# hherlyng/knp-emi-cgx

Hardware: AMD Instinct MI355X
Metric: MDoF/s per implicit timestep (assembly+GMRES) (higher is better)
Workload: dtype f64

## Files before the change

include/knpemi_hip.h:

```cpp
#ifndef KNPEMI_HIP_H
#define KNPEMI_HIP_H

#include <stdint.h>

#ifdef __cplusplus
extern "C" {
#endif

#define KNP_MAX_IONS 3
#define KNP_MAX_AUX 8
#define KNP_DIAG_MAX_CONSTS 64
#define KNP_MAX_PROG_REGS 48
#define KNP_MAX_AMG_LEVELS 16

#define KNP_OK 0
#define KNP_E_ARG (-1)
#define KNP_E_HIP (-2)
#define KNP_E_STATE (-3)
#define KNP_E_ALLOC (-4)
#define KNP_E_MESH (-5)

#define KNP_CONVERGED_RTOL 2
#define KNP_CONVERGED_ATOL 3
#define KNP_DIVERGED_ITS (-3)
// ... 131 lines not shown
int knp_amg_reset(knp_ctx* ctx, int32_t hier, int32_t n_levels, int32_t pre_sweeps, int32_t post_sweeps, int32_t cheby_degree);
int knp_amg_set_node_fields(knp_ctx* ctx, int32_t hier, int32_t nf);
int knp_amg_set_level(knp_ctx* ctx, int32_t hier, int32_t level, int32_t n_rows, int32_t n_cols_halo,
                      const int32_t* A_rowptr, const int32_t* A_colind, const double* A_vals,
                      const double* inv_diag, double lambda_max,
                      int32_t n_coarse,
                      const int32_t* P_rowptr, const int32_t* P_colind, const double* P_vals,
                      const int32_t* R_rowptr, const int32_t* R_colind, const double* R_vals);
int knp_amg_set_level_prolongator(knp_ctx* ctx, int32_t hier, int32_t level, int32_t n_rows_P, const int32_t* P_rp,
                                  const int32_t* P_ci, const double* P_v);
int knp_amg_set_level_mode(knp_ctx* ctx, int32_t hier, int32_t level, int32_t distributed, int32_t repl_n);
int knp_amg_set_coarse(knp_ctx* ctx, int32_t hier, int32_t n, const double* dense_inverse );
int knp_amg_set_level_smoothed(knp_ctx* ctx, int32_t hier, int32_t level, int32_t n_rows, const int32_t* S_rowptr, const int32_t* S_colind,
                        const double* S_vals);
int knp_amg_set_level_coarse_fused(knp_ctx* ctx, int32_t hier, int32_t level, int32_t Rt_rows, const int32_t* Rt_rowptr, const int32_t* Rt_colind,
                                   const double* Rt_vals, int32_t U_rows, const int32_t* U_rowptr, const int32_t* U_colind, const double* U_vals);
int knp_amg_use_native_level0(knp_ctx* ctx, int32_t hier, int32_t mode);
int knp_amg_set_precision(knp_ctx* ctx, int32_t fp32_storage);
int knp_gmres_prepare(knp_ctx* ctx, const double* b);
int knp_gmres_solve(knp_ctx* ctx, const double* b, double* x, double rtol, double atol, int32_t max_it,
                    int32_t restart, int32_t* its, double* rnorm, int32_t* reason);
int knp_fgmres_prepare(knp_ctx* ctx, const double* b);
int knp_fgmres_solve(knp_ctx* ctx, const double* b, double* x, double rtol, double atol, int32_t max_it,
                     int32_t restart, int32_t* its, double* rnorm, int32_t* reason);

int knp_pack(knp_ctx* ctx, const knp_fields_out* fields, double* x);
int knp_unpack(knp_ctx* ctx, const double* x, const knp_fields_out* fields);
int knp_hh_update(knp_ctx* ctx, const double* phi_m, double* n, double* m, double* h, int32_t count,
                  double dt, double phi_rest, int32_t rush_larsen, int32_t substeps);
int knp_l2_norms(knp_ctx* ctx, const double* phi_i, const double* phi_e, double* out );
int knp_diag_set_cell_tags(knp_ctx* ctx, int32_t n_tags, const int32_t* seg_ptr ,
                           const int32_t* cells );
int knp_diag_volume_integrals(knp_ctx* ctx, const knp_fields* fields, double* out );
int knp_diag_set_facet_tags(knp_ctx* ctx, int32_t n_tags, const int32_t* seg_ptr ,
                            const int32_t* facets );
int knp_diag_set_program(knp_ctx* ctx, int32_t n_instr, const int32_t* code , int32_t n_consts,
                         const double* consts );
int knp_diag_set_program_constants(knp_ctx* ctx, int32_t n_consts, const double* consts );
int knp_diag_membrane_integral(knp_ctx* ctx, const knp_fields* fields, double* out );

int knp_timer_mark(knp_ctx* ctx, int32_t join_assembly);
int knp_timer_read(knp_ctx* ctx, int32_t capacity, double* seconds , int32_t* n_intervals);
int knp_timer_pending(const knp_ctx* ctx);
int knp_profile_enable(knp_ctx* ctx, int32_t class_mask);
int knp_profile_get(knp_ctx* ctx, int32_t cls, double* ms, int64_t* launches);
int knp_profile_reset(knp_ctx* ctx);
enum { KNP_ST_BNORM = 0 , KNP_ST_ALLREDUCE = 1 ,
       KNP_ST_HALO = 2 , KNP_ST_READBACK = 3 ,
       KNP_ST_FUSED = 4 ,
       KNP_ST_NORM_FALLBACK = 5 ,
       KNP_ST_BLOCKED = 6 ,
       KNP_ST_FUSED_LEVELS = 7 ,
       KNP_ST_FUSED_DOTS = 8 ,
       KNP_ST_SPMV_DOTS = 9 , KNP_ST_COUNT = 10 };
int knp_get_stats(const knp_ctx* ctx, double* out );
int knp_get_traffic_model(const knp_ctx* ctx, double* out );

#ifdef __cplusplus
}
#endif
#endif
```

knp-emi-cgx_amd/cgx_hip/backend.py:

```python
from __future__ import annotations

import ctypes as C
import os

import numpy as np
import torch

from . import _lib
from ._lib import Fields, FieldsOut, KnpError, MeshDesc
from .parallel import HaloPlan, all_reduce_sum_, guarded


class _CAI:

    def __init__(self, ptr, n):
        self.__cuda_array_interface__ = {"shape": (int(n),), "typestr": "<f8", "data": (int(ptr), False),
                                         "version": 2, "strides": None}


def _f64(a):
    return a.ctypes.data_as(_lib.f64p)


def _i32(a):
# ... 543 lines not shown
        self.check(self.lib.knp_pc_set_coupled_potential(self.ctx, 1 if on else 0))

    def precond_phi_csr(self, embedded=True):
        import scipy.sparse as sp
        sz = (C.c_int64 * _lib.KNP_SZ_COUNT)()
        self.check(self.lib.knp_get_sizes(self.ctx, sz))
        nnz = sz[_lib.SZ_NNZ_P_PHI]
        no = self.n_nodes_owned
        rp = np.empty(no + 1, dtype=np.int32)
        ci = np.empty(nnz, dtype=np.int32)
        va = np.empty(nnz, dtype=np.float64)
        self.check(self.lib.knp_get_precond_phi_csr(self.ctx, _i32(rp), _i32(ci), _f64(va)))
        if not embedded:
            M = sp.csr_matrix((va, ci, rp), shape=(no, self.n_nodes))
            M.sort_indices()
            return M
        keep = va != 0.0
        node_of_entry = np.repeat(np.arange(no, dtype=np.int32), np.diff(rp))
        cnt = np.bincount(node_of_entry[keep], minlength=no)
        indptr = np.zeros(self.n_dof_owned + 1, dtype=np.int64)
        indptr[4 * np.arange(no, dtype=np.int64) + 4] = cnt
        np.cumsum(indptr, out=indptr)
        idx_t = np.int32 if max(int(indptr[-1]), self.n_dof_local) < 2 ** 31 - 1 else np.int64
        M = sp.csr_matrix((va[keep], (4 * ci[keep].astype(idx_t) + 3), indptr.astype(idx_t)), shape=(self.n_dof_owned, self.n_dof_local))
        M.sort_indices()
        return M

    def timer_mark(self, join_assembly=False):
        self.check(self.lib.knp_timer_mark(self.ctx, 1 if join_assembly else 0))

    def timer_pending(self):
        return int(self.lib.knp_timer_pending(self.ctx))

    def timer_read(self):
        n = self.timer_pending()
        if n < 2:
            if n:
                out = (C.c_double * 1)()
                k = C.c_int32()
                self.check(self.lib.knp_timer_read(self.ctx, 1, out, C.byref(k)))
            return np.zeros(0)
        out = (C.c_double * n)()
        k = C.c_int32()
        self.check(self.lib.knp_timer_read(self.ctx, n, out, C.byref(k)))
        return np.array(out[:k.value], dtype=np.float64)

    def profile_enable(self, mask=0x1f):
        self.check(self.lib.knp_profile_enable(self.ctx, int(mask)))

    def profile_reset(self):
        self.check(self.lib.knp_profile_reset(self.ctx))

    def stats(self):
        out = (C.c_double * 10)()
        self.check(self.lib.knp_get_stats(self.ctx, out))
        return {"bnorm": out[0], "allreduces": int(out[1]), "halos": int(out[2]), "readbacks": int(out[3]), "fused": int(out[4]),
                "norm_fallbacks": int(out[5]), "blocked": int(out[6]), "fused_levels": int(out[7]),
                "fused_dots": int(out[8]), "spmv_dots": int(out[9])}

    def traffic_model(self):
        out = (C.c_double * 5)()
        self.check(self.lib.knp_get_traffic_model(self.ctx, out))
        return {"spmv": out[0], "pc": out[1], "assembly_matrix": out[2], "assembly_rhs": out[3], "vector": out[4]}

    def profile_get(self):
        names = ["spmv", "orthogonalisation", "pc", "assembly", "other"]
        out = {}
        for k, nm in enumerate(names):
            ms = C.c_double()
            n = C.c_int64()
            self.check(self.lib.knp_profile_get(self.ctx, k, C.byref(ms), C.byref(n)))
            out[nm] = (ms.value, n.value)
        return out
```

knp-emi-cgx_amd/csrc/knp_internal.hpp:

```cpp
#pragma once
#include <hip/hip_runtime.h>

#include <cstdint>
#include <string>
#include <vector>

#include "knpemi_hip.h"

#define KNP_NPROF 5

struct KnpHostGraph {
    int dim = 0, nv1 = 0;
    int n_v = 0, n_v_owned = 0, n_c = 0, n_c_owned = 0, n_g = 0, n_q = 0;
    int n_nodes = 0, n_nodes_owned = 0;
    std::vector<int32_t> node_i, node_e;
    std::vector<int32_t> node_vertex;
    std::vector<uint8_t> node_side;
    std::vector<int32_t> pair_ptr;
    std::vector<int32_t> pair_col;
    std::vector<int32_t> pair_row;
    std::vector<double> pair_M, pair_K;
    std::vector<int32_t> contrib_ptr;
    std::vector<int32_t> contrib_cell;
    std::vector<double> contrib_k;
// ... 232 lines not shown
    double *d_w = nullptr, *d_t = nullptr;
    double* d_Z = nullptr;
    int z_cap = 0;
    double* d_partial = nullptr;
    double* d_red = nullptr;
    double* h_red = nullptr;
    double* h_red_dev = nullptr;
    double* mirror() const { return (allreduce && p2p_red < 0) ? nullptr : h_red_dev; }
    int64_t phi_count_cached = -1;
    int64_t* h_seq = nullptr;
    int64_t* h_seq_dev = nullptr;
    int64_t seq_counter = 0;
    int asm_full = 0;
    double asm_dt = -1.0;
    int n_bc = 0;
    int32_t* d_bc_dofs = nullptr;
    int defl_m = 0;
    int32_t* d_defl_mode = nullptr;
    double* d_defl_einv = nullptr;
    double* d_y = nullptr;
    double* d_gm = nullptr;
    int gm_cap = 0;
    int64_t n_norm_fallback = 0;
    int n_red_blocks = 0;
    knp_halo_fn halo = nullptr;
    knp_allreduce_fn allreduce = nullptr;
    knp_level_comm_fn level_comm = nullptr;
    void* comm_user = nullptr;
    KnpP2P* p2p = nullptr;
    int p2p_fine = -1;
    int p2p_red = -1;
    bool hook_allreduce() const { return allreduce && p2p_red < 0; }
    int comm_rc = 0;
    int n_int = 0, n_bnd = 0;
    int32_t *d_nodes_int = nullptr, *d_nodes_bnd = nullptr;
    hipStream_t stream3 = nullptr;
    hipEvent_t ev_x = nullptr, ev_halo = nullptr;
    hipStream_t stream2 = nullptr;
    hipEvent_t ev_fork = nullptr, ev_join = nullptr;
    const double* prep_b = nullptr;
    const double* fprep_b = nullptr;
    int prep_fused = 0;
    int prep_conc = 0;
    bool prep_deferred = false;
    bool side_ws = false;
    double *d_t2_s = nullptr, *d_w2_s = nullptr, *d_wb = nullptr, *d_partial_s = nullptr;
    hipStream_t stream_asm = nullptr;
    hipEvent_t ev_fork_asm = nullptr, ev_asm = nullptr;
    bool asm_pending = false;
    double last_bnorm = 0.0;
    int64_t n_allreduce = 0, n_halo = 0, n_readback = 0;
    int64_t n_fused_dots = 0;
    int64_t n_spmv_dots = 0;
    std::vector<hipEvent_t> tm_events;
    size_t tm_used = 0;
    KnpDiagMap diag_cells, diag_facets;
    int32_t* diag_code = nullptr;
    int diag_n_instr = 0, diag_n_regs = 0, diag_n_consts = 0;
    double diag_consts[KNP_DIAG_MAX_CONSTS] = {};
    bool diag_prog = false;
    int prof_on = 0;
    std::vector<hipEvent_t> prof_pool;
    struct ProfRec { hipEvent_t a, b; int cls; };
    std::vector<ProfRec> prof_recs;
    double prof_ms[KNP_NPROF] = {0, 0, 0, 0, 0};
    int64_t prof_n[KNP_NPROF] = {0, 0, 0, 0, 0};
};

int knp_host_threads();
```

knp-emi-cgx_amd/csrc/knp_kernels.hip:

```cpp
#include <hip/hip_runtime.h>
#include <hip/hip_ext.h>

#include <algorithm>
#include <cmath>
#include <cstdio>
#include <cstdlib>
#include <cstring>
#include <new>

#include "knp_internal.hpp"

#define HIPCHK(call)                                                                       \
    do {                                                                                   \
        hipError_t e_ = (call);                                                            \
        if (e_ != hipSuccess) {                                                            \
            ctx->err = std::string(#call) + ": " + hipGetErrorString(e_);                  \
            return KNP_E_HIP;                                                              \
        }                                                                                  \
    } while (0)
#define KCHK(expr)                         \
    do {                                   \
        int rc_ = (expr);                  \
        if (rc_ != KNP_OK) return rc_;     \
    } while (0)
// ... 1829 lines not shown
    a = block_sum(a, sm);
    if (threadIdx.x == 0) {
        out[slot0 + i] = a;
        if (host_mirror) host_mirror[slot0 + i] = a;
        if (seq) {
            __threadfence_system();
            *seq = seq_val;
        }
    }
}

__global__ void __launch_bounds__(NT) k_dot(int n, const double* __restrict__ a, const double* __restrict__ b,
                                            double* __restrict__ partial) {
    __shared__ double sm[NT / 64];
    double acc = 0.0;
    for (int e = blockIdx.x * NT + threadIdx.x; e < n; e += gridDim.x * NT) acc += a[e] * b[e];
    acc = block_sum(acc, sm);
    if (threadIdx.x == 0) partial[blockIdx.x] = acc;
}

__global__ void __launch_bounds__(NT) k_scale_rsqrt(int n, const double* __restrict__ in, const double* __restrict__ nrm2,
                                                    double* __restrict__ out) {
    const double inv = 1.0 / sqrt(*nrm2);
    for (int e = blockIdx.x * NT + threadIdx.x; e < n; e += gridDim.x * NT) out[e] = in[e] * inv;
}
__global__ void __launch_bounds__(NT) k_scale_rsqrt_proj(int n, const double* __restrict__ in, const double* __restrict__ nrm2,
                                                         const double* __restrict__ phi_sum, double inv_count, double* __restrict__ out,
                                                         double* __restrict__ gm_g = nullptr, int m = 0) {
    if (gm_g && blockIdx.x == 0)
        for (int i = threadIdx.x; i <= m; i += NT) gm_g[i] = (i == 0) ? sqrt(*nrm2) : 0.0;
    const double inv = 1.0 / sqrt(*nrm2);
    const double mean = (*phi_sum) * inv_count;
    for (int e = blockIdx.x * NT + threadIdx.x; e < n; e += gridDim.x * NT) out[e] = ((e & 3) == 3 ? in[e] - mean : in[e]) * inv;
}
__global__ void k_proj_norm(double* __restrict__ red, int slot_s, int slot_out, double inv_count, double cancel, double* mirror,
                            volatile int64_t* seq, int64_t seq_val) {
    if (threadIdx.x != 0) return;
    proj_norm_body(red[slot_s], red[slot_s + 1], red, slot_out, inv_count, cancel, mirror, seq, seq_val);
}
__global__ void __launch_bounds__(NT) k_lincomb(int n, int64_t ldv, int m, const double* __restrict__ V,
                                                const double* __restrict__ y, double* __restrict__ x) {
    for (int e = blockIdx.x * NT + threadIdx.x; e < n; e += gridDim.x * NT) {
        double xe = x[e];
        for (int i = 0; i < m; ++i) xe += y[i] * V[(int64_t)i * ldv + e];
        x[e] = xe;
    }
}

__global__ void k_gm_init(GmLayout L, double* __restrict__ gm, const double* __restrict__ beta2) {
    const int t = threadIdx.x;
    for (int i = t; i <= L.m; i += blockDim.x) gm[L.g() + i] = (i == 0) ? sqrt(*beta2) : 0.0;
}

__global__ void __launch_bounds__(NT)
k_update_scale(int n, int64_t ldv, int m, const double* __restrict__ V, const double* __restrict__ h, const double* __restrict__ w,
               const double* __restrict__ st, double ns_scale, double* __restrict__ out) {
    const double inv = st[1] == 0.0 ? 1.0 / sqrt(st[0]) : 1.0;
    const double mean = ns_scale != 0.0 ? h[m] * ns_scale : 0.0;
    const int n2 = n >> 1;
    for (int e2 = blockIdx.x * NT + threadIdx.x; e2 < n2; e2 += gridDim.x * NT) {
        double2 we = *reinterpret_cast<const double2*>(w + 2 * (size_t)e2);
        if (e2 & 1) we.y -= mean;
        for (int i = 0; i < m; ++i) {
            const double2 v = *reinterpret_cast<const double2*>(V + (int64_t)i * ldv + 2 * (size_t)e2);
            const double hi = h[i];
            we.x -= hi * v.x;
            we.y -= hi * v.y;
        }
        *reinterpret_cast<double2*>(out + 2 * (size_t)e2) = make_double2(we.x * inv, we.y * inv);
    }
}
__global__ void __launch_bounds__(NT) k_scale_inplace_rsqrt(int n, const double* __restrict__ nrm2, double* __restrict__ v) {
    const double inv = 1.0 / sqrt(*nrm2);
    for (int e = blockIdx.x * NT + threadIdx.x; e < n; e += gridDim.x * NT) v[e] *= inv;
}
__global__ void k_gm_solve_y(GmLayout L, int jd, double* __restrict__ gm) {
    if (threadIdx.x != 0) return;
    double* y = gm + L.y();
    const double* g = gm + L.g();
    for (int i = jd - 1; i >= 0; --i) {
        double s = g[i];
        for (int k = i + 1; k < jd; ++k) s -= gm[L.H(i, k)] * y[k];
        y[i] = s / gm[L.H(i, i)];
    }
}

__global__ void __launch_bounds__(NT) k_lincomb_solve(GmLayout L, int jd, double* __restrict__ gm, int n, int64_t ldv,
                                                      const double* __restrict__ V, double* __restrict__ x) {
    __shared__ double sH[8 * 8], sg[8], sy[8];
    if (threadIdx.x < jd * jd) sH[threadIdx.x] = gm[L.H(threadIdx.x % jd, threadIdx.x / jd)];
    if (threadIdx.x < jd) sg[threadIdx.x] = gm[L.g() + threadIdx.x];
    __syncthreads();
    if (threadIdx.x == 0) {
        for (int i = jd - 1; i >= 0; --i) {
            double s = sg[i];
            for (int k = i + 1; k < jd; ++k) s -= sH[i + jd * k] * sy[k];
            sy[i] = s / sH[i + jd * i];
        }
        if (blockIdx.x == 0)
            for (int i = 0; i < jd; ++i) gm[L.y() + i] = sy[i];
    }
    __syncthreads();
    for (int e = blockIdx.x * NT + threadIdx.x; e < n; e += gridDim.x * NT) {
        double xe = x[e];
        for (int i = 0; i < jd; ++i) xe += sy[i] * V[(int64_t)i * ldv + e];
        x[e] = xe;
    }
}

template <bool SOLVE>
__global__ void __launch_bounds__(NT) k_zcorr(GmLayout L, int jd, double* __restrict__ gm, int n, int64_t ldv, const double* __restrict__ Z,
                                              double* __restrict__ t, double* __restrict__ partial) {
    __shared__ double sH[8 * 8], sg[8], sy[8], sm[NT / 64];
    if (SOLVE) {
        if (threadIdx.x < jd * jd) sH[threadIdx.x] = gm[L.H(threadIdx.x % jd, threadIdx.x / jd)];
        if (threadIdx.x < jd) sg[threadIdx.x] = gm[L.g() + threadIdx.x];
        __syncthreads();
        if (threadIdx.x == 0) {
            for (int i = jd - 1; i >= 0; --i) {
                double s = sg[i];
                for (int k = i + 1; k < jd; ++k) s -= sH[i + jd * k] * sy[k];
                sy[i] = s / sH[i + jd * i];
            }
            if (blockIdx.x == 0)
                for (int i = 0; i < jd; ++i) gm[L.y() + i] = sy[i];
        }
        __syncthreads();
    }
    const double* __restrict__ y = SOLVE ? sy : gm + L.y();
    double ps = 0.0;
    for (int e = blockIdx.x * NT + threadIdx.x; e < n; e += gridDim.x * NT) {
        double c = 0.0;
        for (int i = 0; i < jd; ++i) c += y[i] * Z[(int64_t)i * ldv + e];
        t[e] = c;
        if ((e & 3) == 3) ps += c;
    }
    ps = block_sum(ps, sm);
    if (threadIdx.x == 0) partial[blockIdx.x] = ps;
}
__global__ void __launch_bounds__(NT) k_axpy_proj(int n, const double* __restrict__ t, const double* __restrict__ phi_sum, double inv_count,
                                                  double* __restrict__ x) {
    const double mean = (*phi_sum) * inv_count;
    for (int e = blockIdx.x * NT + threadIdx.x; e < n; e += gridDim.x * NT) x[e] += (e & 3) == 3 ? t[e] - mean : t[e];
}

__global__ void __launch_bounds__(NT) k_axpy(int n, double a, const double* __restrict__ x, double* __restrict__ y) {
    for (int e = blockIdx.x * NT + threadIdx.x; e < n; e += gridDim.x * NT) y[e] += a * x[e];
}
__global__ void __launch_bounds__(NT) k_fill(int n, double a, double* __restrict__ y) {
    for (int e = blockIdx.x * NT + threadIdx.x; e < n; e += gridDim.x * NT) y[e] = a;
}
__global__ void __launch_bounds__(NT) k_diag_scale(int n, double a, const double* __restrict__ d,
                                                   const double* __restrict__ x, double* __restrict__ y) {
    for (int e = blockIdx.x * NT + threadIdx.x; e < n; e += gridDim.x * NT) y[e] = a * d[e] * x[e];
}

__global__ void __launch_bounds__(NT) k_phi_sum(int n_nodes, const double* __restrict__ z, double* __restrict__ partial) {
    __shared__ double sm[NT / 64];
    double acc = 0.0;
    for (int n = blockIdx.x * NT + threadIdx.x; n < n_nodes; n += gridDim.x * NT) acc += z[(size_t)4 * n + 3];
// ... 2641 lines not shown
        HIPCHK(hipMemset(ctx->d_gm, 0, (size_t)GL.size() * sizeof(double)));
        ctx->gm_cap = GL.size();
    }
    double* gm = ctx->d_gm;
    auto read_state = [&](double& res_out, int& flag_out) -> int {
        ++ctx->n_readback;
        if (ctx->mirror() && ctx->h_seq_dev) {
            KCHK(read_slots_inner(ctx, GM_RES, 2, ctx->seq_counter));
            if (ctx->p2p) KCHK(knp_p2p_check(ctx));
            res_out = ctx->h_red[GM_RES];
            flag_out = (int)ctx->h_red[GM_RES + 1];
        } else {
            double tmp[3];
            HIPCHK(hipMemcpyAsync(tmp, gm + GL.st(), 3 * sizeof(double), hipMemcpyDeviceToHost, st));
            HIPCHK(hipStreamSynchronize(st));
            res_out = tmp[2];
            flag_out = (int)tmp[1];
        }
        return KNP_OK;
    };

    bool lazy_bnorm = false;
    if (ctx->prep_b == b && restart == ctx->gm_restart && ctx->prep_conc) {
        lazy_bnorm = true;
    } else if (ctx->prep_b == b && restart == ctx->gm_restart) {
        HIPCHK(hipEventSynchronize(ctx->ev_join));
        ctx->prep_b = nullptr;
        if (!ctx->h_red_dev) {
            HIPCHK(hipMemcpy(ctx->h_red + 60, ctx->d_red + 60, 2 * sizeof(double), hipMemcpyDeviceToHost));
        }
        if (ctx->prep_fused && ctx->h_red[61] != 0.0) {
            ++ctx->n_norm_fallback;
            KCHK(pc_apply_proj(ctx, b, ctx->d_w, cnt));
            KCHK(dot_to_slot(ctx, ctx->d_w, ctx->d_w, 60));
            KCHK(read_slots(ctx, 60, 1, ctx->seq_counter));
        }
    } else {
        side_discard(ctx);
        bool fused_norm = false;
        KCHK(pc_apply_norm(ctx, b, ctx->d_w, cnt, &fused_norm));
        KCHK(pc_norm_read(ctx, ctx->d_w, cnt, &fused_norm));
    }
    double bnorm = lazy_bnorm ? 0.0 : std::sqrt(ctx->h_red[60]);
    ctx->last_bnorm = bnorm;
    if (!lazy_bnorm && !std::isfinite(bnorm)) { *its = 0; *rnorm = bnorm; *reason = KNP_DIVERGED_NANORINF; return KNP_OK; }
    double ttol = std::max(rtol * bnorm, atol);
    const double dtol = 1e5;
    int it = 0;
    double res = 0.0, res0 = -1.0;
    *reason = 0;
    const bool ns = ctx->ns_on && cnt > 0;
    const int nsi = ns ? 1 : 0;
    const int vec_blocks = std::min(nblocks(n), 2048);
    while (true) {
        KCHK(spmv_A(ctx, x, b, ctx->d_t, true));
        bool fused_norm = false;
        KCHK(pc_apply_norm(ctx, ctx->d_t, ctx->d_w, cnt, &fused_norm));
        if (lazy_bnorm && ctx->prep_deferred) {
            ctx->prep_deferred = false;
            HIPCHK(hipStreamWaitEvent(ctx->stream2, ctx->ev_fork, 0));
            ctx->stream = ctx->stream2;
            bool fn = false;
            swap_side_ws(ctx);
            const int rcs = pc_apply_norm(ctx, b, ctx->d_wb, cnt, &fn, true);
            swap_side_ws(ctx);
            ctx->stream = st;
            KCHK(rcs);
            HIPCHK(hipEventRecord(ctx->ev_join, ctx->stream2));
        }
        KCHK(pc_norm_read(ctx, ctx->d_w, cnt, &fused_norm));
        if (lazy_bnorm) {
            lazy_bnorm = false;
            HIPCHK(hipEventSynchronize(ctx->ev_join));
            ctx->prep_b = nullptr;
            double nb2 = ctx->h_red[SIDE_SLOT];
            if (ctx->h_red[SIDE_SLOT + 1] != 0.0) {
                ++ctx->n_norm_fallback;
                KCHK(pc_apply_proj(ctx, b, ctx->d_wb, cnt));
                KCHK(dot_to_slot(ctx, ctx->d_wb, ctx->d_wb, 60));
                KCHK(read_slots(ctx, 60, 1, ctx->seq_counter));
                nb2 = ctx->h_red[60];
                KCHK(pc_apply_norm(ctx, ctx->d_t, ctx->d_w, cnt, &fused_norm));
                KCHK(pc_norm_read(ctx, ctx->d_w, cnt, &fused_norm));
            }
            bnorm = std::sqrt(nb2);
            ctx->last_bnorm = bnorm;
            if (!std::isfinite(bnorm)) { *its = 0; *rnorm = bnorm; *reason = KNP_DIVERGED_NANORINF; return KNP_OK; }
            ttol = std::max(rtol * bnorm, atol);
        }
        const double beta = std::sqrt(ctx->h_red[60]);
        res = beta;
        if (res0 < 0) res0 = beta;
        if (!std::isfinite(beta)) { *reason = KNP_DIVERGED_NANORINF; break; }
        if (beta <= ttol) { *reason = (beta <= atol) ? KNP_CONVERGED_ATOL : KNP_CONVERGED_RTOL; break; }
        if (it >= max_it) { *reason = KNP_DIVERGED_ITS; break; }
        if (fused_norm) {
            hipLaunchKernelGGL(k_scale_rsqrt_proj, dim3(vec_blocks), dim3(NT), 0, st, n, ctx->d_w, ctx->d_red + 60, ctx->d_red + 62,
                               1.0 / (double)cnt, ctx->d_V, gm + GL.g(), m);
        } else {
            hipLaunchKernelGGL(k_scale_rsqrt, dim3(vec_blocks), dim3(NT), 0, st, n, ctx->d_w, ctx->d_red + 60, ctx->d_V);
            hipLaunchKernelGGL(k_gm_init, dim3(1), dim3(64), 0, st, GL, gm, ctx->d_red + 60);
        }
        int jd = 0;
        bool stop = false;
        for (int j = 0; j < m; ++j) {
            double* vj = ctx->d_V + (size_t)j * ldv;
            double* vn = ctx->d_V + (size_t)(j + 1) * ldv;
            KCHK(spmv_A(ctx, vj, nullptr, ctx->d_t, false));
            DotReq dq{j + 1, ns, ldv, ctx->d_V, ctx->d_partial};
            KCHK(pc_apply_proj(ctx, ctx->d_t, ctx->d_w, ns ? 0 : cnt, (ctx->fused_dots && fin_ok(ctx) && j + 1 <= BU_MAX_M) ? &dq : nullptr));
            int flag = 0;
            {
                ProfScope ps(ctx, 1);
                const int nbr = dq.done ? dq.nb : nb;
                const int pst = dq.done ? RED_WIDE : RED_BLOCKS;
                for (int i0 = 0; i0 <= j && !dq.done; i0 += 8) {
                    if (i0 == 0 && ns)
                        hipLaunchKernelGGL((k_multi_dot<8, true, true>), dim3(nb), dim3(NT), 0, st, n, ldv, i0, j + 1, ctx->d_V, ctx->d_w, ctx->d_partial);
                    else if (i0 == 0)
                        hipLaunchKernelGGL((k_multi_dot<8, false, true>), dim3(nb), dim3(NT), 0, st, n, ldv, i0, j + 1, ctx->d_V, ctx->d_w, ctx->d_partial);
                    else
                        hipLaunchKernelGGL((k_multi_dot<8, false, false>), dim3(nb), dim3(NT), 0, st, n, ldv, i0, j + 1, ctx->d_V, ctx->d_w, ctx->d_partial);
                }
                const int nred = j + 2 + nsi;
                if (fin_ok(ctx)) {
                    ++ctx->n_allreduce;
                    hipLaunchKernelGGL(k_reduce_fin, dim3(1), dim3(NT), 0, st, 1, nbr, nred, ctx->d_partial, ctx->d_red, 0, GL, j, nsi, ns ? 1.0 / (double)cnt : 0.0, gm,
                                       0, 0.0, ctx->mirror() ? ctx->h_red_dev + GM_RES : nullptr, ctx->mirror() ? ctx->h_seq_dev : nullptr, ++ctx->seq_counter,
                                       pst);
                } else {
                    hipLaunchKernelGGL(k_reduce_partials, dim3(nred), dim3(NT), 0, st, nbr, ctx->d_partial, ctx->d_red, 0, (double*)nullptr);
                    KCHK(allreduce_slots(ctx, 0, nred));
                    hipLaunchKernelGGL(k_givens, dim3(1), dim3(64), 0, st, GL, j, nsi, ns ? 1.0 / (double)cnt : 0.0, ctx->d_red, -1, gm,
                                       ctx->mirror() ? ctx->h_red_dev + GM_RES : nullptr, ctx->mirror() ? ctx->h_seq_dev : nullptr, ++ctx->seq_counter);
                }
                hipLaunchKernelGGL(k_update_scale, dim3(nb), dim3(NT), 0, st, n, ldv, j + 1, ctx->d_V, ctx->d_red, ctx->d_w, gm + GL.st(),
                                   ns ? 1.0 / (double)cnt : 0.0, vn);
                HIPCHK(hipGetLastError());
            }
            KCHK(read_state(res, flag));
            if (flag == 1) {
                ProfScope ps(ctx, 1);
                ++ctx->n_norm_fallback;
                hipLaunchKernelGGL(k_dot, dim3(nb), dim3(NT), 0, st, n, vn, vn, ctx->d_partial);
                hipLaunchKernelGGL(k_reduce_partials, dim3(1), dim3(NT), 0, st, nb, ctx->d_partial, ctx->d_red, GM_EXPL, (double*)nullptr);
                KCHK(allreduce_slots(ctx, GM_EXPL, 1));
                hipLaunchKernelGGL(k_givens, dim3(1), dim3(64), 0, st, GL, j, nsi, ns ? 1.0 / (double)cnt : 0.0, ctx->d_red, GM_EXPL, gm,
                                   ctx->mirror() ? ctx->h_red_dev + GM_RES : nullptr, ctx->mirror() ? ctx->h_seq_dev : nullptr, ++ctx->seq_counter);
                hipLaunchKernelGGL(k_scale_inplace_rsqrt, dim3(vec_blocks), dim3(NT), 0, st, n, gm + GL.st(), vn);
                HIPCHK(hipGetLastError());
                KCHK(read_state(res, flag));
            }
            if (flag != 0 || !std::isfinite(res)) { *reason = KNP_DIVERGED_NANORINF; stop = true; jd = j; break; }
            ++it;
            jd = j + 1;
            if (res <= ttol) { *reason = (res <= atol) ? KNP_CONVERGED_ATOL : KNP_CONVERGED_RTOL; stop = true; break; }
            if (it >= max_it) { *reason = KNP_DIVERGED_ITS; stop = true; break; }
            if (res > dtol * res0) { *reason = KNP_DIVERGED_DTOL; stop = true; break; }
        }
        if (jd > 0) {
            ProfScope ps(ctx, 1);
            if (jd <= 8) {
                hipLaunchKernelGGL(k_lincomb_solve, dim3(vec_blocks), dim3(NT), 0, st, GL, jd, gm, n, ldv, ctx->d_V, x);
            } else {
                hipLaunchKernelGGL(k_gm_solve_y, dim3(1), dim3(64), 0, st, GL, jd, gm);
                hipLaunchKernelGGL(k_lincomb, dim3(vec_blocks), dim3(NT), 0, st, n, ldv, jd, ctx->d_V, gm + GL.y(), x);
            }
        }
        if (stop) break;
    }
    *its = it;
    *rnorm = res;
    KCHK(halo_update(ctx, x));
    HIPCHK(hipGetLastError());
    if (ctx->p2p) {
        HIPCHK(hipStreamSynchronize(st));
        KCHK(knp_p2p_check(ctx));
    }
    if (ctx->comm_rc != KNP_OK) { const int rc2 = ctx->comm_rc; ctx->comm_rc = KNP_OK; return rc2; }
    return KNP_OK;
}

static constexpr int FB_SLOT = 124;
static int ensure_z(knp_ctx* ctx, int restart) {
    if (ctx->d_Z && ctx->z_cap >= restart) return KNP_OK;
    HIPCHK(hipStreamSynchronize(ctx->stream));
    dev_free(ctx->d_Z);
    const size_t bytes = (size_t)restart * std::max(ctx->n_dof_local, 1) * sizeof(double);
    HIPCHK(hipMalloc((void**)&ctx->d_Z, bytes));
    HIPCHK(hipMemset(ctx->d_Z, 0, bytes));
    ctx->z_cap = restart;
    return KNP_OK;
}

int knp_fgmres_prepare(knp_ctx* ctx, const double* b) {
    CHECK_CTX(ctx);
    if (!b) return KNP_E_ARG;
    side_discard(ctx);
    if (getenv("KNP_NO_PREPARE") || (ctx->prof_on & ~1) || ctx->halo || ctx->allreduce || ctx->level_comm || ctx->p2p) return KNP_OK;
    if (!ctx->stream2) {
        HIPCHK(hipStreamCreateWithFlags(&ctx->stream2, hipStreamNonBlocking));
        HIPCHK(hipEventCreateWithFlags(&ctx->ev_fork, hipEventDisableTiming));
        HIPCHK(hipEventCreateWithFlags(&ctx->ev_join, hipEventDisableTiming));
    }
    if (!ctx->d_partial_s) {
        HIPCHK(hipMalloc((void**)&ctx->d_partial_s, (size_t)RED_SLOTS * RED_BLOCKS * sizeof(double)));
        HIPCHK(hipMemset(ctx->d_partial_s, 0, (size_t)RED_SLOTS * RED_BLOCKS * sizeof(double)));
    }
    const int nb = ctx->n_red_blocks;
    HIPCHK(hipEventRecord(ctx->ev_fork, ctx->stream));
    HIPCHK(hipStreamWaitEvent(ctx->stream2, ctx->ev_fork, 0));
    hipLaunchKernelGGL(k_dot, dim3(nb), dim3(NT), 0, ctx->stream2, ctx->n_dof_owned, b, b, ctx->d_partial_s);
    hipLaunchKernelGGL(k_reduce_partials, dim3(1), dim3(NT), 0, ctx->stream2, nb, ctx->d_partial_s, ctx->d_red, FB_SLOT, ctx->mirror(),
// ... 243 lines not shown
}

int knp_timer_mark(knp_ctx* ctx, int32_t join_assembly) {
    CHECK_CTX(ctx);
    if (join_assembly) KCHK(join_asm(ctx));
    if (ctx->tm_used == ctx->tm_events.size()) {
        hipEvent_t e = nullptr;
        HIPCHK(hipEventCreate(&e));
        ctx->tm_events.push_back(e);
    }
    HIPCHK(hipEventRecord(ctx->tm_events[ctx->tm_used++], ctx->stream));
    return KNP_OK;
}
int knp_timer_read(knp_ctx* ctx, int32_t capacity, double* seconds, int32_t* n_intervals) {
    CHECK_CTX(ctx);
    if (!seconds || !n_intervals || capacity < 0) return KNP_E_ARG;
    const size_t n = ctx->tm_used;
    *n_intervals = 0;
    if (n == 0) return KNP_OK;
    if ((size_t)capacity + 1 < n) { ctx->err = "knp_timer_read: capacity below the number of marks - 1"; return KNP_E_ARG; }
    HIPCHK(hipEventSynchronize(ctx->tm_events[n - 1]));
    for (size_t i = 0; i + 1 < n; ++i) {
        float ms = 0.f;
        HIPCHK(hipEventElapsedTime(&ms, ctx->tm_events[i], ctx->tm_events[i + 1]));
        seconds[i] = 1e-3 * (double)ms;
    }
    *n_intervals = (int32_t)(n - 1);
    ctx->tm_used = 0;
    return KNP_OK;
}
int knp_timer_pending(const knp_ctx* ctx) { return ctx ? (int)ctx->tm_used : 0; }

int knp_profile_enable(knp_ctx* ctx, int32_t on) {
    CHECK_CTX(ctx);
    KCHK(prof_collect(ctx));
    ctx->prof_on = on;
    return KNP_OK;
}
int knp_profile_get(knp_ctx* ctx, int32_t cls, double* ms, int64_t* launches) {
    CHECK_CTX(ctx);
    if (cls < 0 || cls >= KNP_NPROF || !ms || !launches) return KNP_E_ARG;
    KCHK(prof_collect(ctx));
    *ms = ctx->prof_ms[cls];
    *launches = ctx->prof_n[cls];
    return KNP_OK;
}
int knp_profile_reset(knp_ctx* ctx) {
    CHECK_CTX(ctx);
    KCHK(prof_collect(ctx));
    for (int i = 0; i < KNP_NPROF; ++i) { ctx->prof_ms[i] = 0; ctx->prof_n[i] = 0; }
    ctx->n_allreduce = ctx->n_halo = ctx->n_readback = ctx->n_norm_fallback = 0;
    ctx->n_fused_dots = 0;
    ctx->n_spmv_dots = 0;
    return KNP_OK;
}
static double cycle_bytes(const knp_ctx* ctx, const KnpAmgHier& H) {
    if (H.levels < 1) return 0.0;
    const double vs = H.cinv_f || ctx->amg_fp32 ? 4.0 : 8.0;
    double b = 0.0;
    const int nl = H.levels;
    const int nf0 = H.native0 == 1 ? 4 : H.native0 == 2 ? 3 : 1;
    const double n0 = (double)ctx->g.n_nodes_owned;
    auto blocked = [&](const KnpBlockedCsr& M, int nf) { return (double)M.nnz * (nf == 4 ? 20.0 : 16.0) + 4.0 * (M.n_rows + 1); };
    auto scalar = [&](int64_t nnz, int rows) { return (double)nnz * (vs + 4.0) + 4.0 * (rows + 1); };
    if (H.at0_rp) b += scalar(H.lv[0].A_nnz, ctx->g.n_nodes_owned);
    else if (H.native0) b += (double)ctx->n_pairs * (vs * nf0 + 4.0) + 4.0 * (n0 + 1);
    else b += scalar(H.lv[0].A_nnz, H.lv[0].n);
    b += 8.0 * n0 * nf0 * 3.0;
    for (int l = 0; l < nl - 1; ++l) {
        const KnpAmgLevel& L = H.lv[l];
        const double nl_ = (double)(l == 0 ? n0 * nf0 : L.n), nc_ = (double)L.n_coarse;
        const bool mid = l >= 1 && H.cfused;
        if (mid) {
            b += (H.blocked ? blocked(L.bRt, H.node_nf) : scalar(L.Rt_nnz, L.n_coarse)) + 8.0 * (nl_ + nc_);
            b += (H.blocked ? blocked(L.bU, H.node_nf) : scalar(L.U_nnz, L.n)) + 8.0 * (nl_ + nc_ + nl_);
        } else {
            b += (H.blocked ? blocked(L.bR, H.node_nf) : scalar(L.R_nnz, L.n_coarse)) + 8.0 * (nl_ + nc_);
            b += (H.blocked ? blocked(L.bS, H.node_nf) : scalar(L.S_nnz, L.n)) + 8.0 * (nc_ + 4.0 * nl_);
            if (l >= 1) b += (H.blocked ? blocked(L.bA, H.node_nf) : scalar(L.A_nnz, L.n)) + 8.0 * 3.0 * nl_;
        }
    }
    if (H.nc > 0) b += (double)H.nc * H.nc * (H.cinv_f ? 4.0 : 8.0) + 16.0 * H.nc;
    return b;
}
int knp_get_traffic_model(const knp_ctx* ctx, double* out) {
    if (!ctx || !out) return KNP_E_ARG;
    const KnpHostGraph& g = ctx->g;
    const double np_ = (double)ctx->n_pairs, no = (double)g.n_nodes_owned, ngp = (double)ctx->n_gp;
    static const bool mf_off = getenv("KNP_SPMV_MF") && atoi(getenv("KNP_SPMV_MF")) == 0;
    const bool mf = !mf_off && ctx->n_bc == 0 && ctx->d_pair_MK != nullptr;
    out[0] = np_ * (32.0 + (mf ? 16.0 : 48.0) + 4.0) + no * (4.0 + 4.0 + 1.0) + 2.0 * ngp * (32.0 + 4.0) + 8.0 * ctx->n_dof_owned + 8.0 * ctx->n_dof_local;
    double pc = 0.0;
    if (ctx->pc_kind == KNP_PC_AMG) pc = cycle_bytes(ctx, ctx->hier[0]);
    else if (ctx->pc_kind == KNP_PC_AMG_BT || ctx->pc_kind == KNP_PC_AMG_LT)
        pc = cycle_bytes(ctx, ctx->hier[0]) + cycle_bytes(ctx, ctx->hier[1]) + np_ * 12.0 + no * 8.0 * 9.0;
    else if (ctx->pc_kind == KNP_PC_VBJACOBI) pc = no * 8.0 * (16.0 + 8.0);
    out[1] = pc;
    const double conc = ctx->asm_dmax > 0 ? (double)g.n_nodes * 56.0 + np_ * 36.0 + (double)ctx->n_node_cells * g.nv1
                                          : (double)g.n_c * (4.0 * g.nv1 + 32.0 + 24.0 * g.nv1) + (double)ctx->n_node_cells * 36.0;
    out[2] = (double)(ctx->n_tc > 0 ? ctx->n_tc : ctx->n_contrib) * 9.0 + conc + np_ * 32.0 + ngp * (64.0 + 48.0);
    out[3] = no * (8.0 * 4.0 + 9.0) + np_ * (8.0 + 4.0 + 24.0) + (double)g.n_g * g.dim * 7.0 * 8.0 * 2.0;
    out[4] = 8.0 * ctx->n_dof_owned;
    return KNP_OK;
}
int knp_get_stats(const knp_ctx* ctx, double* out) {
    if (!ctx || !out) return KNP_E_ARG;
    for (int i = 0; i < KNP_ST_COUNT; ++i) out[i] = 0.0;
    out[KNP_ST_BNORM] = ctx->last_bnorm;
    out[KNP_ST_ALLREDUCE] = (double)ctx->n_allreduce;
    out[KNP_ST_HALO] = (double)ctx->n_halo;
    out[KNP_ST_READBACK] = (double)ctx->n_readback;
    out[KNP_ST_FUSED] = (double)(ctx->hier[0].fused + 2 * ctx->hier[1].fused + 4 * ctx->hier[0].l0_fused + 8 * ctx->hier[1].l0_fused);
    out[KNP_ST_NORM_FALLBACK] = (double)ctx->n_norm_fallback;
    out[KNP_ST_BLOCKED] = (double)(ctx->hier[0].blocked + 2 * ctx->hier[1].blocked);
    int nlf = 0;
    for (int h = 0; h < KNP_MAX_HIER; ++h)
        for (int l = 1; l < ctx->hier[h].levels; ++l) nlf += ctx->hier[h].lv[l].lfused;
    out[KNP_ST_FUSED_LEVELS] = (double)nlf;
    out[KNP_ST_FUSED_DOTS] = (double)ctx->n_fused_dots;
    out[KNP_ST_SPMV_DOTS] = (double)ctx->n_spmv_dots;
    return KNP_OK;
}

}

#include "knp_diagnostics.inc"
```

Baseline: 2184.

## Speculatively enqueue GMRES cycle start and finish solution update on device

Before the host reads back the initial residual norm, the first normalisation and SpMV of each GMRES cycle are now enqueued speculatively, so the GPU keeps working while the host-side convergence check runs. If convergence or a norm fallback makes the speculation invalid, the results are discarded. The update kernel can also do the small triangular solve and the x update on the device once the residual is already below tolerance (m<=8), which removes a separate lincomb launch. Both paths are single-GPU only, can be disabled with environment variables, and add wasted work when speculation is dropped.

Measured after the change: 2248, median of 6. 2.9% higher.

```diff
diff --git a/include/knpemi_hip.h b/include/knpemi_hip.h
--- a/include/knpemi_hip.h
+++ b/include/knpemi_hip.h
@@ -207,7 +207,11 @@
        KNP_ST_BLOCKED = 6 ,
        KNP_ST_FUSED_LEVELS = 7 ,
        KNP_ST_FUSED_DOTS = 8 ,
-       KNP_ST_SPMV_DOTS = 9 , KNP_ST_COUNT = 10 };
+       KNP_ST_SPMV_DOTS = 9 ,
+       KNP_ST_SPEC_ENTRY = 10 ,
+       KNP_ST_SPEC_DROPPED = 11 ,
+       KNP_ST_DEV_FINISH = 12 ,
+       KNP_ST_COUNT = 13 };
 int knp_get_stats(const knp_ctx* ctx, double* out );
 int knp_get_traffic_model(const knp_ctx* ctx, double* out );
 
diff --git a/knp-emi-cgx_amd/cgx_hip/backend.py b/knp-emi-cgx_amd/cgx_hip/backend.py
--- a/knp-emi-cgx_amd/cgx_hip/backend.py
+++ b/knp-emi-cgx_amd/cgx_hip/backend.py
@@ -619,11 +619,12 @@
         self.check(self.lib.knp_profile_reset(self.ctx))
 
     def stats(self):
-        out = (C.c_double * 10)()
+        out = (C.c_double * 13)()
         self.check(self.lib.knp_get_stats(self.ctx, out))
         return {"bnorm": out[0], "allreduces": int(out[1]), "halos": int(out[2]), "readbacks": int(out[3]), "fused": int(out[4]),
                 "norm_fallbacks": int(out[5]), "blocked": int(out[6]), "fused_levels": int(out[7]),
-                "fused_dots": int(out[8]), "spmv_dots": int(out[9])}
+                "fused_dots": int(out[8]), "spmv_dots": int(out[9]),
+                "spec_entries": int(out[10]), "spec_dropped": int(out[11]), "dev_finishes": int(out[12])}
 
     def traffic_model(self):
         out = (C.c_double * 5)()
diff --git a/knp-emi-cgx_amd/csrc/knp_internal.hpp b/knp-emi-cgx_amd/csrc/knp_internal.hpp
--- a/knp-emi-cgx_amd/csrc/knp_internal.hpp
+++ b/knp-emi-cgx_amd/csrc/knp_internal.hpp
@@ -308,6 +308,8 @@
     int64_t n_allreduce = 0, n_halo = 0, n_readback = 0;
     int64_t n_fused_dots = 0;
     int64_t n_spmv_dots = 0;
+    int64_t n_spec_entry = 0, n_spec_dropped = 0;
+    int64_t n_dev_finish = 0;
     std::vector<hipEvent_t> tm_events;
     size_t tm_used = 0;
     KnpDiagMap diag_cells, diag_facets;
diff --git a/knp-emi-cgx_amd/csrc/knp_kernels.hip b/knp-emi-cgx_amd/csrc/knp_kernels.hip
--- a/knp-emi-cgx_amd/csrc/knp_kernels.hip
+++ b/knp-emi-cgx_amd/csrc/knp_kernels.hip
@@ -1905,9 +1905,36 @@
     for (int i = t; i <= L.m; i += blockDim.x) gm[L.g() + i] = (i == 0) ? sqrt(*beta2) : 0.0;
 }
 
+__device__ __forceinline__ void lincomb_solve_body(GmLayout L, int jd, double* __restrict__ gm, int n, int64_t ldv, const double* __restrict__ V,
+                                                   double* __restrict__ x, double* sH, double* sg, double* sy) {
+    if (threadIdx.x < jd * jd) sH[threadIdx.x] = gm[L.H(threadIdx.x % jd, threadIdx.x / jd)];
+    if (threadIdx.x < jd) sg[threadIdx.x] = gm[L.g() + threadIdx.x];
+    __syncthreads();
+    if (threadIdx.x == 0) {
+        for (int i = jd - 1; i >= 0; --i) {
+            double s = sg[i];
+            for (int k = i + 1; k < jd; ++k) s -= sH[i + jd * k] * sy[k];
+            sy[i] = s / sH[i + jd * i];
+        }
+        if (blockIdx.x == 0)
+            for (int i = 0; i < jd; ++i) gm[L.y() + i] = sy[i];
+    }
+    __syncthreads();
+    for (int e = blockIdx.x * NT + threadIdx.x; e < n; e += gridDim.x * NT) {
+        double xe = x[e];
+        for (int i = 0; i < jd; ++i) xe += sy[i] * V[(int64_t)i * ldv + e];
+        x[e] = xe;
+    }
+}
 __global__ void __launch_bounds__(NT)
 k_update_scale(int n, int64_t ldv, int m, const double* __restrict__ V, const double* __restrict__ h, const double* __restrict__ w,
-               const double* __restrict__ st, double ns_scale, double* __restrict__ out) {
+               const double* __restrict__ st, double ns_scale, double* __restrict__ out, double ttol = -1.0, GmLayout L = GmLayout{1},
+               double* __restrict__ gm = nullptr, double* __restrict__ x = nullptr) {
+    __shared__ double sH[8 * 8], sg[8], sy[8];
+    if (ttol >= 0.0 && m <= 8 && st[1] == 0.0 && st[2] <= ttol) {
+        lincomb_solve_body(L, m, gm, n, ldv, V, x, sH, sg, sy);
+        return;
+    }
     const double inv = st[1] == 0.0 ? 1.0 / sqrt(st[0]) : 1.0;
     const double mean = ns_scale != 0.0 ? h[m] * ns_scale : 0.0;
     const int n2 = n >> 1;
@@ -1941,24 +1968,7 @@
 __global__ void __launch_bounds__(NT) k_lincomb_solve(GmLayout L, int jd, double* __restrict__ gm, int n, int64_t ldv,
                                                       const double* __restrict__ V, double* __restrict__ x) {
     __shared__ double sH[8 * 8], sg[8], sy[8];
-    if (threadIdx.x < jd * jd) sH[threadIdx.x] = gm[L.H(threadIdx.x % jd, threadIdx.x / jd)];
-    if (threadIdx.x < jd) sg[threadIdx.x] = gm[L.g() + threadIdx.x];
-    __syncthreads();
-    if (threadIdx.x == 0) {
-        for (int i = jd - 1; i >= 0; --i) {
-            double s = sg[i];
-            for (int k = i + 1; k < jd; ++k) s -= sH[i + jd * k] * sy[k];
-            sy[i] = s / sH[i + jd * i];
-        }
-        if (blockIdx.x == 0)
-            for (int i = 0; i < jd; ++i) gm[L.y() + i] = sy[i];
-    }
-    __syncthreads();
-    for (int e = blockIdx.x * NT + threadIdx.x; e < n; e += gridDim.x * NT) {
-        double xe = x[e];
-        for (int i = 0; i < jd; ++i) xe += sy[i] * V[(int64_t)i * ldv + e];
-        x[e] = xe;
-    }
+    lincomb_solve_body(L, jd, gm, n, ldv, V, x, sH, sg, sy);
 }
 
 template <bool SOLVE>
@@ -4706,10 +4716,27 @@
     const bool ns = ctx->ns_on && cnt > 0;
     const int nsi = ns ? 1 : 0;
     const int vec_blocks = std::min(nblocks(n), 2048);
+    const bool spec_off = getenv("KNP_SPEC_ENTRY") && atoi(getenv("KNP_SPEC_ENTRY")) == 0;
+    const bool devfin_off = getenv("KNP_DEV_FINISH") && atoi(getenv("KNP_DEV_FINISH")) == 0;
+    const bool one_gpu = !ctx->halo && !ctx->allreduce && !ctx->level_comm && !ctx->p2p;
+    const bool spec_entry = !spec_off && one_gpu && max_it > 0;
+    const bool dev_fin = !devfin_off && one_gpu && fin_ok(ctx);
+    auto start_cycle = [&](bool fused_norm) {
+        if (fused_norm) {
+            hipLaunchKernelGGL(k_scale_rsqrt_proj, dim3(vec_blocks), dim3(NT), 0, st, n, ctx->d_w, ctx->d_red + 60, ctx->d_red + 62,
+                               1.0 / (double)cnt, ctx->d_V, gm + GL.g(), m);
+        } else {
+            hipLaunchKernelGGL(k_scale_rsqrt, dim3(vec_blocks), dim3(NT), 0, st, n, ctx->d_w, ctx->d_red + 60, ctx->d_V);
+            hipLaunchKernelGGL(k_gm_init, dim3(1), dim3(64), 0, st, GL, gm, ctx->d_red + 60);
+        }
+    };
     while (true) {
         KCHK(spmv_A(ctx, x, b, ctx->d_t, true));
         bool fused_norm = false;
         KCHK(pc_apply_norm(ctx, ctx->d_t, ctx->d_w, cnt, &fused_norm));
+        bool spec = false;
+        int64_t spec_halos = 0;
+        auto drop_spec = [&]() { if (spec) ++ctx->n_spec_dropped; ctx->n_halo -= spec_halos; spec_halos = 0; spec = false; };
         if (lazy_bnorm && ctx->prep_deferred) {
             ctx->prep_deferred = false;
             HIPCHK(hipStreamWaitEvent(ctx->stream2, ctx->ev_fork, 0));
@@ -4722,7 +4749,17 @@
             KCHK(rcs);
             HIPCHK(hipEventRecord(ctx->ev_join, ctx->stream2));
         }
+        const bool fused_at_launch = fused_norm;
+        if (spec_entry && it < max_it) {
+            start_cycle(fused_norm);
+            const int64_t h0 = ctx->n_halo;
+            KCHK(spmv_A(ctx, ctx->d_V, nullptr, ctx->d_t, false));
+            spec_halos = ctx->n_halo - h0;
+            spec = true;
+            ++ctx->n_spec_entry;
+        }
         KCHK(pc_norm_read(ctx, ctx->d_w, cnt, &fused_norm));
+        if (fused_norm != fused_at_launch) drop_spec();
         if (lazy_bnorm) {
             lazy_bnorm = false;
             HIPCHK(hipEventSynchronize(ctx->ev_join));
@@ -4734,33 +4771,33 @@
                 KCHK(dot_to_slot(ctx, ctx->d_wb, ctx->d_wb, 60));
                 KCHK(read_slots(ctx, 60, 1, ctx->seq_counter));
                 nb2 = ctx->h_red[60];
+                if (spec_entry && it < max_it) {
+                    const int64_t h1 = ctx->n_halo;
+                    KCHK(spmv_A(ctx, x, b, ctx->d_t, true));
+                    ctx->n_halo = h1;
+                }
+                drop_spec();
                 KCHK(pc_apply_norm(ctx, ctx->d_t, ctx->d_w, cnt, &fused_norm));
                 KCHK(pc_norm_read(ctx, ctx->d_w, cnt, &fused_norm));
             }
             bnorm = std::sqrt(nb2);
             ctx->last_bnorm = bnorm;
-            if (!std::isfinite(bnorm)) { *its = 0; *rnorm = bnorm; *reason = KNP_DIVERGED_NANORINF; return KNP_OK; }
+            if (!std::isfinite(bnorm)) { drop_spec(); *its = 0; *rnorm = bnorm; *reason = KNP_DIVERGED_NANORINF; return KNP_OK; }
             ttol = std::max(rtol * bnorm, atol);
         }
         const double beta = std::sqrt(ctx->h_red[60]);
         res = beta;
         if (res0 < 0) res0 = beta;
-        if (!std::isfinite(beta)) { *reason = KNP_DIVERGED_NANORINF; break; }
-        if (beta <= ttol) { *reason = (beta <= atol) ? KNP_CONVERGED_ATOL : KNP_CONVERGED_RTOL; break; }
-        if (it >= max_it) { *reason = KNP_DIVERGED_ITS; break; }
-        if (fused_norm) {
-            hipLaunchKernelGGL(k_scale_rsqrt_proj, dim3(vec_blocks), dim3(NT), 0, st, n, ctx->d_w, ctx->d_red + 60, ctx->d_red + 62,
-                               1.0 / (double)cnt, ctx->d_V, gm + GL.g(), m);
-        } else {
-            hipLaunchKernelGGL(k_scale_rsqrt, dim3(vec_blocks), dim3(NT), 0, st, n, ctx->d_w, ctx->d_red + 60, ctx->d_V);
-            hipLaunchKernelGGL(k_gm_init, dim3(1), dim3(64), 0, st, GL, gm, ctx->d_red + 60);
-        }
+        if (!std::isfinite(beta)) { drop_spec(); *reason = KNP_DIVERGED_NANORINF; break; }
+        if (beta <= ttol) { drop_spec(); *reason = (beta <= atol) ? KNP_CONVERGED_ATOL : KNP_CONVERGED_RTOL; break; }
+        if (it >= max_it) { drop_spec(); *reason = KNP_DIVERGED_ITS; break; }
+        if (!spec) start_cycle(fused_norm);
         int jd = 0;
-        bool stop = false;
+        bool stop = false, x_done = false;
         for (int j = 0; j < m; ++j) {
             double* vj = ctx->d_V + (size_t)j * ldv;
             double* vn = ctx->d_V + (size_t)(j + 1) * ldv;
-            KCHK(spmv_A(ctx, vj, nullptr, ctx->d_t, false));
+            if (!(spec && j == 0)) KCHK(spmv_A(ctx, vj, nullptr, ctx->d_t, false));
             DotReq dq{j + 1, ns, ldv, ctx->d_V, ctx->d_partial};
             KCHK(pc_apply_proj(ctx, ctx->d_t, ctx->d_w, ns ? 0 : cnt, (ctx->fused_dots && fin_ok(ctx) && j + 1 <= BU_MAX_M) ? &dq : nullptr));
             int flag = 0;
@@ -4789,10 +4826,11 @@
                                        ctx->mirror() ? ctx->h_red_dev + GM_RES : nullptr, ctx->mirror() ? ctx->h_seq_dev : nullptr, ++ctx->seq_counter);
                 }
                 hipLaunchKernelGGL(k_update_scale, dim3(nb), dim3(NT), 0, st, n, ldv, j + 1, ctx->d_V, ctx->d_red, ctx->d_w, gm + GL.st(),
-                                   ns ? 1.0 / (double)cnt : 0.0, vn);
+                                   ns ? 1.0 / (double)cnt : 0.0, vn, dev_fin ? ttol : -1.0, GL, gm, x);
                 HIPCHK(hipGetLastError());
             }
             KCHK(read_state(res, flag));
+            x_done = dev_fin && j + 1 <= 8 && flag == 0 && res <= ttol;
             if (flag == 1) {
                 ProfScope ps(ctx, 1);
                 ++ctx->n_norm_fallback;
@@ -4812,7 +4850,8 @@
             if (it >= max_it) { *reason = KNP_DIVERGED_ITS; stop = true; break; }
             if (res > dtol * res0) { *reason = KNP_DIVERGED_DTOL; stop = true; break; }
         }
-        if (jd > 0) {
+        if (x_done) ++ctx->n_dev_finish;
+        if (jd > 0 && !x_done) {
             ProfScope ps(ctx, 1);
             if (jd <= 8) {
                 hipLaunchKernelGGL(k_lincomb_solve, dim3(vec_blocks), dim3(NT), 0, st, GL, jd, gm, n, ldv, ctx->d_V, x);
@@ -5162,6 +5201,7 @@
     ctx->n_allreduce = ctx->n_halo = ctx->n_readback = ctx->n_norm_fallback = 0;
     ctx->n_fused_dots = 0;
     ctx->n_spmv_dots = 0;
+    ctx->n_spec_entry = ctx->n_spec_dropped = ctx->n_dev_finish = 0;
     return KNP_OK;
 }
 static double cycle_bytes(const knp_ctx* ctx, const KnpAmgHier& H) {
@@ -5229,6 +5269,9 @@
     out[KNP_ST_FUSED_LEVELS] = (double)nlf;
     out[KNP_ST_FUSED_DOTS] = (double)ctx->n_fused_dots;
     out[KNP_ST_SPMV_DOTS] = (double)ctx->n_spmv_dots;
+    out[KNP_ST_SPEC_ENTRY] = (double)ctx->n_spec_entry;
+    out[KNP_ST_SPEC_DROPPED] = (double)ctx->n_spec_dropped;
+    out[KNP_ST_DEV_FINISH] = (double)ctx->n_dev_finish;
     return KNP_OK;
 }
 
```
